# jyjblrd/Low-Cost-Mocap

Hardware: AMD Instinct MI355X
Metric: triangulated 3D markers/sec at 8 cams x 16 markers (higher is better)
Workload: dtype f64

## Files before the change

### low-cost-mocap_amd/csrc/frame_bb.hip

```cpp
#include "mocap_device.hpp"
#include "kernels.hpp"
#include <cstdlib>
#include "frame_common.hpp"

namespace mocap {

constexpr int kBBThreads = 256;
constexpr int kBBWaves = kBBThreads / 64;
constexpr int kBBRecs = kBBThreads + 64;

constexpr int bb_wg_per_cu(int RL) { return RL == 48 ? 5 : 4; }
constexpr int kBBLdsSlack = 1024;
struct BBLayout {
  size_t bxy, bxy_nx, cnt_nx, bt, rbound, seedkey, slot_key, claimw, recs, rpk, scr, scr_bytes, goff, gcnt, outslot, boff, bnb, seedgh, slot_g, cnt,
      misc, bpl, nh, hits, act, root_blob, root_cam, nact, bnl, bv, bcache, bpk, total;
  int ncache;
  __host__ __device__ static size_t al(size_t x, size_t a) { return (x + a - 1) / a * a; }
  __host__ __device__ BBLayout(int C, int M, int R, int CW, int wg_per_cu) {
    size_t o = 0;
    auto take = [&](size_t bytes, size_t a) {
      o = al(o, a);
      const size_t at = o;
      o += bytes;
      return at;
    };
    bxy = take(sizeof(float2) * (size_t)C * M, 16);
    bxy_nx = take(sizeof(float2) * (size_t)C * M, 16);
    cnt_nx = take(4 * (size_t)C, 4);
    bt = take(sizeof(double) * 10 * ((size_t)C * M + 1), 16);
    rbound = take(8 * (size_t)R, 8);
    claimw = take(8 * (size_t)C, 8);
    scr = seedkey = take(8 * (size_t)R, 8);
    slot_key = take(8 * (size_t)kBBWaves * R, 8);
    recs = take(8 * (size_t)kBBRecs, 8);
    rpk = take(8 * (size_t)kBBRecs * CW, 8);
    seedgh = take(4 * (size_t)R, 4);
    slot_g = take(4 * (size_t)kBBWaves * R, 4);
    scr_bytes = o - scr;
    goff = take(4 * (size_t)(R + 1), 4);
    gcnt = take(4 * (size_t)R, 4);
    outslot = take(4 * (size_t)R, 4);
    boff = take(4 * (size_t)(R + 1), 4);
    bnb = take(4 * (size_t)R, 4);
    cnt = take(4 * (size_t)C, 4);
    misc = take(4 * 16, 4);
    bpl = take(2 * (size_t)R, 2);
    nh = take((size_t)R * C, 1);
    hits = take((size_t)R * C * M, 1);
    act = take((size_t)R * C, 1);
    root_blob = take((size_t)R, 1);
    root_cam = take((size_t)R, 1);
    nact = take((size_t)R, 1);
    bnl = take((size_t)R, 1);
    bv = take((size_t)R, 1);
    bcache = take(0, 8);
    ncache = 0;
    const size_t per_entry = 8 + 8 * (size_t)CW;
    for (int per_cu = wg_per_cu; per_cu >= 1; per_cu--) {
      const size_t lim = ((size_t)160 * 1024 / per_cu - kBBLdsSlack) / 256 * 256;
      if (lim >= o + per_entry * 64) {
        const size_t n = (lim - o) / per_entry;
        ncache = (int)(n > 1024 ? 1024 : n);
        break;
      }
    }
    o += 8 * (size_t)ncache;
    bpk = o;
    o += 8 * (size_t)CW * ncache;
    total = al(o, 16);
  }
};

static int bb_fixed_slots(int C, int M, int R) {
  const char* e = getenv("MOCAP_BB_FIXED_LAYOUT");
  if (e && e[0] == '0') return 0;
  if (C == 8 && M == 16 && R <= 48) return 48;
  if (C == 8 && M == 16 && R <= 64) return 64;
  return 0;
}
static int frame_bb_root_slots(int C, int M, int R) {
  const int f = bb_fixed_slots(C, M, R);
  return f ? f : R;
}
size_t frame_bb_lds_bytes(int C, int M, int R) { return BBLayout(C, M, frame_bb_root_slots(C, M, R), C <= 8 ? 1 : 2, bb_wg_per_cu(bb_fixed_slots(C, M, R))).total; }
static size_t frame_bb_lds_bytes_min(int C, int M, int R) {
  const BBLayout L(C, M, frame_bb_root_slots(C, M, R), C <= 8 ? 1 : 2, bb_wg_per_cu(bb_fixed_slots(C, M, R)));
  return L.total - (8 + 8 * (size_t)(C <= 8 ? 1 : 2)) * (size_t)L.ncache;
}
bool frame_bb_fits(int C, int M, int R) {
  return C >= 2 && C <= 16 && M >= 1 && M <= 64 && R >= 1 && R <= 255 && frame_bb_lds_bytes_min(C, M, R) <= (size_t)128 * 1024;
}

template <int CW>
struct Packed {
  unsigned long long w[CW];
  __device__ __forceinline__ void clear() {
#pragma unroll
    for (int k = 0; k < CW; k++) w[k] = ~0ull;
  }
  __device__ __forceinline__ void set(int c, uint32_t idx) {
    if (CW == 1)
      w[0] ^= (unsigned long long)(idx ^ 0xFFu) << (8 * c);
    else
      w[c >> 3] ^= (unsigned long long)(idx ^ 0xFFu) << (8 * (c & 7));
  }
  __device__ __forceinline__ uint32_t get(int c) const {
    return CW == 1 ? (uint32_t)(w[0] >> (8 * c)) & 0xFFu : (uint32_t)(w[c >> 3] >> (8 * (c & 7))) & 0xFFu;
  }
};

template <int CT, bool PERK = false>
struct BBCamTables {
  const double* base;
  static constexpr int C = CT;
  static constexpr int kPq = PERK ? 12 * CT * CT : 12 * CT;
  __device__ __forceinline__ ctab_t pq(size_t off) const { return as_ctab(base + off); }
  __device__ __forceinline__ ctab_t rt(size_t off) const { return as_ctab(base + kPq + off); }
  __device__ __forceinline__ ctab_t k4(size_t off) const { return as_ctab(base + kPq + 12 * CT + off); }
  __device__ __forceinline__ const double* f() const { return base + kPq + 16 * CT; }
};
template <bool PERK>
struct BBCamTables<0, PERK> {
  const double* base;
  int C;
  __device__ __forceinline__ ctab_t pq(size_t off) const { return as_ctab(base + off); }
  __device__ __forceinline__ ctab_t rt(size_t off) const { return as_ctab(base + (PERK ? 12 * C * C : 12 * C) + off); }
  __device__ __forceinline__ ctab_t k4(size_t off) const { return as_ctab(base + (PERK ? 12 * C * C + 12 * C : 24 * C) + off); }
  __device__ __forceinline__ const double* f() const { return base + (PERK ? 12 * C * C + 16 * C : 28 * C); }
};

enum { kPrioEval = 0, kPrioSeed = 1, kPrioPhase = 2, kPrioSerial = 3 };
template <int P>
__device__ __forceinline__ void bb_prio() {
  __builtin_amdgcn_s_setprio(P);
}

template <bool F32R, int CW, int CT, int ML, int RL, bool PERK = false>
struct BBState {
  static constexpr int T = kBBThreads, W = kBBWaves;
  const FrameArgs& p;
  BBCamTables<CT, PERK> cv;
  const int C_, M, R, RS;
  int tid, lane, wave;
  __device__ __forceinline__ void fresh_tid() {
    int t = tid;
    asm volatile("" : "+v"(t));
    tid = t;
    lane = t & 63;
    wave = t >> 6;
  }
  __device__ __forceinline__ int cn() const { return CT > 0 ? CT : C_; }
  double* bt;
  float2 *bxy, *bxy_nx;
  int32_t* cnt_nx;
  unsigned long long *rbound, *seedkey, *slot_key, *claimw, *rpk;
  struct BRec { uint32_t gh, rs; };
  BRec* recs;
  uint32_t *goff, *gcnt, *boff, *bnb, *seedgh, *slot_g;
  int32_t *outslot, *cnt, *misc;
  uint16_t* bpl;
  uint8_t *nh, *hits, *act, *root_blob, *root_cam, *nact, *bnl, *bv;
  float2* bcache;
  unsigned long long* bpk;
  int ncache;
  unsigned char* scr;
  size_t scr_bytes;
  static constexpr unsigned long long kInfBits = 0x7ff0000000000000ull;

  __device__ BBState(const FrameArgs& p_, unsigned char* smem)
      : p(p_), C_(p_.cv.C), M(ML > 0 ? ML : p_.M), R(p_.K_max), RS(RL > 0 ? RL : p_.K_max), tid(threadIdx.x), lane(threadIdx.x & 63), wave(threadIdx.x >> 6) {
    const int C = cn();
    {
      const unsigned long long ta = (unsigned long long)(uintptr_t)p_.cv.Pq;
      uint32_t tlo = (uint32_t)__builtin_amdgcn_readfirstlane((int)(uint32_t)ta);
      uint32_t thi = (uint32_t)__builtin_amdgcn_readfirstlane((int)(uint32_t)(ta >> 32));
      asm volatile("" : "+s"(tlo), "+s"(thi));
      cv.base = (const double*)(uintptr_t)(((unsigned long long)thi << 32) | tlo);
      if constexpr (CT == 0) cv.C = C;
    }
    const BBLayout L(C, M, RS, CW, bb_wg_per_cu(RL));
    bt = (double*)(smem + L.bt);
    bxy = (float2*)(smem + L.bxy);
    bxy_nx = (float2*)(smem + L.bxy_nx);
    cnt_nx = (int32_t*)(smem + L.cnt_nx);
    rbound = (unsigned long long*)(smem + L.rbound);
    seedkey = (unsigned long long*)(smem + L.seedkey);
    slot_key = (unsigned long long*)(smem + L.slot_key);
    claimw = (unsigned long long*)(smem + L.claimw);
    recs = (BRec*)(smem + L.recs);
    rpk = (unsigned long long*)(smem + L.rpk);
    goff = (uint32_t*)(smem + L.goff);
    gcnt = (uint32_t*)(smem + L.gcnt);
    outslot = (int32_t*)(smem + L.outslot);
    boff = (uint32_t*)(smem + L.boff);
    bnb = (uint32_t*)(smem + L.bnb);
    seedgh = (uint32_t*)(smem + L.seedgh);
    slot_g = (uint32_t*)(smem + L.slot_g);
    cnt = (int32_t*)(smem + L.cnt);
    misc = (int32_t*)(smem + L.misc);
    bpl = (uint16_t*)(smem + L.bpl);
    nh = (uint8_t*)(smem + L.nh);
    hits = (uint8_t*)(smem + L.hits);
    act = (uint8_t*)(smem + L.act);
    root_blob = (uint8_t*)(smem + L.root_blob);
    root_cam = (uint8_t*)(smem + L.root_cam);
    nact = (uint8_t*)(smem + L.nact);
    bnl = (uint8_t*)(smem + L.bnl);
    bv = (uint8_t*)(smem + L.bv);
    scr = smem + L.scr;
    scr_bytes = L.scr_bytes;
    bcache = (float2*)(smem + L.bcache);
    bpk = (unsigned long long*)(smem + L.bpk);
    ncache = L.ncache;
  }

  struct Line { double a, b, c, den, rden; };
  __device__ __forceinline__ Line epiline(int r, int i) const { return epiline_of(root_cam[r], root_blob[r], i); }
  __device__ __forceinline__ Line epiline_of(int rc, int rb, int i) const {
    const int C = cn();
    const double* Fm = cv.f() + 9 * ((size_t)rc * C + i);
    const float2 rp = bxy[(size_t)rc * M + rb];
    const double x = (double)rp.x, y = (double)rp.y;
    double a = Fm[0] * x + Fm[1] * y + Fm[2];
    double b = Fm[3] * x + Fm[4] * y + Fm[5];
    double c = Fm[6] * x + Fm[7] * y + Fm[8];
    double nu = a * a + b * b;
    nu = nu != 0.0 ? 1.0 / sqrt(nu) : 1.0;
    a *= nu;
    b *= nu;
    c *= nu;
    if (F32R) {
      a = (double)(float)a;
      b = (double)(float)b;
      c = (double)(float)c;
    }
    Line L;
    L.a = a;
    L.b = b;
    L.c = c;
    L.den = sqrt(a * a + b * b);
    L.rden = recip_refined(L.den);
    return L;
  }

  template <bool CHAIN>
  __device__ __forceinline__ unsigned long long match_pairs(const Line& mine, int pair_r, int pair_i, int n_pairs, int gs_shift,
                                                            int cam = 0, int Mi_chain = 0) {
    const int C = cn();
    const int GS = 1 << gs_shift, PPS = 64 >> gs_shift;
    const int k = lane & (GS - 1), q = lane >> gs_shift;
    const int gl0 = lane & ~(GS - 1);
    const unsigned long long gall = gs_shift == 6 ? ~0ull : ((1ull << GS) - 1ull);
    unsigned long long claims = 0ull;
    for (int s0 = 0; s0 < n_pairs; s0 += PPS) {
      const int src = s0 + q;
      const bool has = src < n_pairs;
      const int sl = has ? src : 0;
      const double la = __shfl(mine.a, sl), lb = __shfl(mine.b, sl), lc = __shfl(mine.c, sl);
      const double lden = __shfl(mine.den, sl), lrden = __shfl(mine.rden, sl);
      const int r = __shfl(pair_r, sl);
      const int i = CHAIN ? cam : __shfl(pair_i, sl);
      const int Mi = has ? (CHAIN ? Mi_chain : cnt[i]) : 0;
      const bool valid = k < Mi;
      float2 pt = make_float2(0.f, 0.f);
      double d = 0.0;
      bool hit = false;
      if (valid) {
        pt = bxy[(size_t)i * M + k];
        const double num = fabs(la * (double)pt.x + lb * (double)pt.y + lc);
        d = div_by(num, lden, lrden);
        hit = d < p.gate_px;
      }
      const unsigned long long wm = __ballot(hit);
      const unsigned long long gm = (wm >> gl0) & gall;
      int rank = 0;
      const unsigned int dlo = (unsigned int)__double_as_longlong(d), dhi = (unsigned int)(__double_as_longlong(d) >> 32);
      for (unsigned long long mm = wm; mm;) {
        const int j = __ffsll((long long)mm) - 1;
        mm &= mm - 1;
        const double dj = __longlong_as_double(((long long)__builtin_amdgcn_readlane((int)dhi, j) << 32) |
                                               (unsigned int)__builtin_amdgcn_readlane((int)dlo, j));
        const bool mine_grp = (j & ~(GS - 1)) == gl0 && j != lane;
        rank += (hit && mine_grp && (dj < d || (dj == d && j < lane))) ? 1 : 0;
      }
      if (hit) hits[((size_t)r * C + i) * M + rank] = (uint8_t)k;
      const unsigned long long g0 = (__ballot(hit && rank == 0) >> gl0) & gall;
      bool same = false;
      if (valid && g0) {
        const float2 p0 = bxy[(size_t)i * M + (__ffsll((long long)g0) - 1)];
        same = pt.x == p0.x && pt.y == p0.y;
      }
      const unsigned long long cw = __ballot(same);
      if (CHAIN) {
        for (int sh = 0; sh < 64; sh += GS) claims |= (cw >> sh) & gall;
      }
      if (has && k == 0) {
        nh[(size_t)r * C + i] = (uint8_t)__popcll(gm);
        if (!CHAIN) {
          const unsigned long long cm = (cw >> gl0) & gall;
          if (cm) atomicOr(&claimw[i], cm);
        }
      }
    }
    return claims;
  }

  __device__ __forceinline__ void prefetch_lds(int64_t frame) const {
    const int C = cn();
    const float* src = p.blobs + (size_t)frame * C * M * 2;
    const int n_dw = C * M * 2;
    for (int base = wave * 64; base < n_dw; base += T)
      if (base + lane < n_dw)
        __builtin_amdgcn_global_load_lds((const __attribute__((address_space(1))) void*)(src + base + lane),
                                         (__attribute__((address_space(3))) void*)((float*)bxy_nx + base), 4, 0, 0);
    if (wave == 0 && lane < C)
      __builtin_amdgcn_global_load_lds((const __attribute__((address_space(1))) void*)(p.counts + (size_t)frame * C + lane),
                                       (__attribute__((address_space(3))) void*)cnt_nx, 4, 0, 0);
  }
  __device__ __forceinline__ void stage(int64_t frame) {
    fresh_tid();
    const int C = cn();
    float2* t = bxy;
    bxy = bxy_nx;
    bxy_nx = t;
    if (tid < C) {
      const int n = cnt_nx[tid];
      cnt[tid] = n < 0 ? 0 : (n > M ? M : n);
      claimw[tid] = 0ull;
    }
    if (tid == 0) {
      misc[MI_STATUS] = 0;
      misc[MI_OMAX] = 0;
    }
  }

  __device__ void match() {
    fresh_tid();
    const int C = cn();
    __syncthreads();
    int gs_shift = 0;
    while ((1 << gs_shift) < M) gs_shift++;
    const int n0 = cnt[0] < R ? cnt[0] : R;
    {
      for (int r = tid; r < n0; r += T) {
        root_cam[r] = 0;
        root_blob[r] = (uint8_t)r;
      }
      if (tid == 0 && cnt[0] > R) misc[MI_STATUS] |= MOCAP_ST_ROOT_OVERFLOW_;
    }
    __syncthreads();
    auto U_of = [&](int j) {
      const int n = cnt[j];
      return ~claimw[j] & (n >= 64 ? ~0ull : ((1ull << n) - 1ull));
    };
    int n_prov = 0, n_ppairs = 0;
    bool pre = false;
    uint8_t* nh_s = nullptr;
    uint8_t* hits_s = nullptr;
    unsigned long long* pclaim = (unsigned long long*)scr;
    {
      int Mmax = 0;
      for (int c = 1; c < C; c++) Mmax = cnt[c] > Mmax ? cnt[c] : Mmax;
#pragma nounroll
      for (int stage_ = 0; stage_ < 2; stage_++) {
        const int stage = __builtin_amdgcn_readfirstlane(stage_);
        int NP = n0 * (C - 1);
        if (stage == 1) {
          block_sync_lds();
          for (int j = 1; j < C; j++) {
            const int np = __popcll(U_of(j));
            n_prov += np;
            n_ppairs += np * (C - 1 - j);
          }
          pre = n_prov <= 64 && (size_t)n_prov * C * (8 + 1 + (size_t)M) <= scr_bytes;
          if (!pre) break;
          nh_s = (uint8_t*)(pclaim + (size_t)n_prov * C);
          hits_s = nh_s + (size_t)n_prov * C;
          NP = n_ppairs;
        }
        for (int base = wave * 64; base < NP; base += W * 64) {
          const int pi = base + lane;
          const bool have = pi < NP;
          int r = 0, i = 1, Mi = 0;
          Line L = {0, 0, 0, 1, 1};
          if (have) {
            if (stage == 0) {
              r = pi / (C - 1);
              i = 1 + (pi - r * (C - 1));
              L = epiline(r, i);
            } else {
              int j = 1, acc = 0, pb = 0, span = C - 2;
              unsigned long long U = 0ull;
              for (; j <= C - 2; j++) {
                span = C - 1 - j;
                U = U_of(j);
                const int nj = __popcll(U) * span;
                if (pi < acc + nj) break;
                acc += nj;
                pb += __popcll(U);
              }
              uint32_t ord, off;
              divmod_tiny((uint32_t)(pi - acc), (uint32_t)span, ord, off);
              for (uint32_t t = 0; t < ord; t++) U &= U - 1;
              const int k = __ffsll((long long)U) - 1;
              i = j + 1 + (int)off;
              r = pb + (int)ord;
              L = epiline_of(j, k, i);
            }
            Mi = cnt[i];
          }
          const float2* pts = bxy + (size_t)i * M;
          auto dist = [&](int k) {
            const float2 pt = pts[k];
            return div_by(fabs(L.a * (double)pt.x + L.b * (double)pt.y + L.c), L.den, L.rden);
          };
          unsigned long long hm = 0ull;
#pragma unroll 4
          for (int k = 0; k < Mmax; k++)
            if (k < Mi && dist(k) < p.gate_px) hm |= 1ull << k;
          uint8_t* nhp = stage == 0 ? nh : nh_s;
          uint8_t* hl = (stage == 0 ? hits : hits_s) + ((size_t)r * C + i) * M;
          if (have) nhp[(size_t)r * C + i] = (uint8_t)__popcll(hm);
          unsigned long long rem = hm, claim = 0ull;
          int pos = 0;
          float2 p0 = make_float2(0.f, 0.f);
          while (__ballot(rem != 0ull)) {
            if (rem) {
              double bd = __builtin_huge_val();
              int bk = 0;
              for (unsigned long long t = rem; t; t &= t - 1) {
                const int k = __ffsll((long long)t) - 1;
                const double d = dist(k);
                if (d < bd) {
                  bd = d;
                  bk = k;
                }
              }
              hl[pos] = (uint8_t)bk;
              if (pos == 0) {
                p0 = pts[bk];
                for (unsigned long long t = hm; t; t &= t - 1) {
                  const int k = __ffsll((long long)t) - 1;
                  const float2 q = pts[k];
                  if (q.x == p0.x && q.y == p0.y) claim |= 1ull << k;
                }
              }
              rem &= ~(1ull << bk);
              pos++;
            }
          }
          if (stage == 0) {
            if (claim) atomicOr(&claimw[i], claim);
          } else if (have) {
            pclaim[(size_t)r * C + i] = claim;
          }
        }
      }
    }
    const int NL = M * ((C - 1) * (C - 2) / 2);
    const bool spec = F32R && (size_t)NL * 20 + 8 <= scr_bytes;
    double* sp_den = (double*)scr;
    float* sp_abc = (float*)(sp_den + NL);
    auto sp_base = [&](int j) { return M * ((j - 1) * (C - 1) - (j - 1) * j / 2); };
    if (spec && !pre) {
      int tot = 0;
      for (int j = 1; j <= C - 2; j++) {
        const int n = cnt[j];
        const unsigned long long U = ~claimw[j] & (n >= 64 ? ~0ull : ((1ull << n) - 1ull));
        tot += __popcll(U) * (C - 1 - j);
      }
      for (int l = tid; l < tot; l += T) {
        int j = 1, acc = 0, span = C - 2;
        unsigned long long U = 0ull;
        for (; j <= C - 2; j++) {
          const int n = cnt[j];
          U = ~claimw[j] & (n >= 64 ? ~0ull : ((1ull << n) - 1ull));
          span = C - 1 - j;
          const int nj = __popcll(U) * span;
          if (l < acc + nj) break;
          acc += nj;
        }
        uint32_t ord, off;
        divmod_tiny((uint32_t)(l - acc), (uint32_t)span, ord, off);
        for (uint32_t t = 0; t < ord; t++) U &= U - 1;
        const int k = __ffsll((long long)U) - 1, i = j + 1 + (int)off;
        const int ll = sp_base(j) + k * span + (int)off;
        const Line L = epiline_of(j, k, i);
        sp_den[ll] = L.den;
        sp_abc[3 * ll + 0] = (float)L.a;
        sp_abc[3 * ll + 1] = (float)L.b;
        sp_abc[3 * ll + 2] = (float)L.c;
      }
    }
    __syncthreads();
    fresh_tid();
    if (wave == 0) bb_prio<kPrioSerial>();
    if (wave == 0 && pre) {
      int jp = 0, kp = 0;
      if (lane < n_prov) {
        int acc = 0;
        unsigned long long U = 0ull;
        for (jp = 1; jp < C; jp++) {
          U = U_of(jp);
          const int np = __popcll(U);
          if (lane < acc + np) break;
          acc += np;
        }
        for (int t = 0; t < lane - acc; t++) U &= U - 1;
        kp = __ffsll((long long)U) - 1;
      }
      bool real = false;
      for (int i = 1; i < C; i++) {
        wave_lds_sync();
        if (lane < n_prov && jp == i) {
          real = !((claimw[i] >> kp) & 1ull);
          if (real)
            for (int c = i + 1; c < C; c++) {
              const unsigned long long m = pclaim[(size_t)lane * C + c];
              if (m) atomicOr(&claimw[c], m);
            }
        }
      }
      const unsigned long long rm = __ballot(real);
      const int rank = __popcll(rm & ((1ull << lane) - 1ull));
      int n_roots = n0 + __popcll(rm);
      if (real && n0 + rank < R) {
        root_cam[n0 + rank] = (uint8_t)jp;
        root_blob[n0 + rank] = (uint8_t)kp;
        bnl[rank] = (uint8_t)lane;
      }
      if (lane == 0) {
        if (n_roots > R) {
          misc[MI_STATUS] |= MOCAP_ST_ROOT_OVERFLOW_;
          n_roots = R;
        }
        misc[MI_NROOTS] = n_roots;
      }
    } else if (wave == 0) {
      const int cntL = lane < C ? cnt[lane] : 0;
      const unsigned long long clmL = lane < C ? claimw[lane] : 0ull;
      int nr_cam = 0, nr_blob = 0;
      int n_roots = n0;
      bool over = false;
      for (int i = 1; i < C; i++) {
        const int Mi = __builtin_amdgcn_readlane(cntL, i);
        unsigned long long claimed = ((unsigned long long)(unsigned int)__builtin_amdgcn_readlane((int)(clmL >> 32), i) << 32) |
                                     (unsigned int)__builtin_amdgcn_readlane((int)clmL, i);
        const int n_new = n_roots - n0;
        for (int base = 0; base < n_new; base += 64) {
          const int l = base + lane;
          const bool have = l < n_new;
          int j = nr_cam, k = nr_blob;
          if (base) {
            wave_lds_sync();
            j = have ? root_cam[n0 + l] : 0;
            k = have ? root_blob[n0 + l] : 0;
          }
          Line L = {0, 0, 0, 1, 1};
          if (have) {
            if (spec) {
              const int ll = sp_base(j) + k * (C - 1 - j) + (i - j - 1);
              L.a = (double)sp_abc[3 * ll + 0];
              L.b = (double)sp_abc[3 * ll + 1];
              L.c = (double)sp_abc[3 * ll + 2];
              L.den = sp_den[ll];
              L.rden = recip_refined(L.den);
            } else {
              L = epiline_of(j, k, i);
            }
          }
          claimed |= match_pairs<true>(L, n0 + l, i, (n_new - base < 64) ? n_new - base : 64, gs_shift, i, Mi);
        }
        const bool flag = lane < Mi && !((claimed >> lane) & 1ull);
        const unsigned long long mask = __ballot(flag);
        const int pos = __popcll(mask & ((1ull << lane) - 1ull));
        if (flag) {
          const int rr = n_roots + pos;
          if (rr < R) {
            root_cam[rr] = (uint8_t)i;
            root_blob[rr] = (uint8_t)lane;
          }
        }
        int slot = n_new;
        for (unsigned long long mm = mask; mm; slot++) {
          const int jb = __ffsll((long long)mm) - 1;
          mm &= mm - 1;
          if (lane == slot) {
            nr_cam = i;
            nr_blob = jb;
          }
        }
        n_roots += __popcll(mask);
        if (n_roots > R) {
          over = true;
          n_roots = R;
        }
      }
      if (lane == 0) {
        if (over) misc[MI_STATUS] |= MOCAP_ST_ROOT_OVERFLOW_;
        misc[MI_NROOTS] = n_roots;
      }
    } else {
      float om = 0.0f;
      for (int i = tid - 64; i < C * M; i += T - 64) {
        const int c = i / M, k = i - c * M;
        if (k < cnt[c]) {
          const float2 v = bxy[i];
          om = fmaxf(om, fmaxf(fabsf(v.x), fabsf(v.y)));
          double Bc[10];
          dlt_contribution(Bc, cv.pq(PERK ? 12 * (c * C + c) : 12 * c), (double)v.x, (double)v.y);
#pragma unroll
          for (int e = 0; e < 10; e++) bt[(size_t)i * 10 + e] = Bc[e];
        }
      }
      if (om > 0.0f) atomicMax(&misc[MI_OMAX], __float_as_int(om));
      if (tid == 64) {
        const int it = q_add(&p.q.counters[QC_NEXT_FRAME], 1);
        misc[MI_NEXT] = it < frame_count(p) ? it : -1;
      }
    }
    bb_prio<kPrioPhase>();
    __syncthreads();
    if (pre) {
      const int n_new = misc[MI_NROOTS] - n0;
      for (int idx = tid; idx < n_new * C; idx += T) {
        const int q = idx / C, c = idx - q * C;
        const int r = n0 + q, ps = bnl[q];
        if (c > (int)root_cam[r]) {
          const int n = nh_s[(size_t)ps * C + c];
          nh[(size_t)r * C + c] = (uint8_t)n;
          const uint8_t* src = hits_s + ((size_t)ps * C + c) * M;
          uint8_t* dst = hits + ((size_t)r * C + c) * M;
          for (int t = 0; t < n; t++) dst[t] = src[t];
        }
      }
      __syncthreads();
    }

    fresh_tid();
    const int nroots = misc[MI_NROOTS];
    for (int r = tid; r < nroots; r += T) {
      const int rc = root_cam[r];
      unsigned long long total = 1;
      int views = 1, na = 0;
      bool over = false;
      for (int c = rc + 1; c < C; c++) {
        const unsigned n = nh[(size_t)r * C + c];
        if (n > 1) act[(size_t)r * C + na++] = (uint8_t)c;
        if (n) {
          views++;
          total *= n;
          if (total > (unsigned long long)p.G_cap) {
            over = true;
            total = 1;
          }
        }
      }
      if (over) atomicOr(&misc[MI_STATUS], MOCAP_ST_CAND_OVERFLOW_);
      nact[r] = (uint8_t)na;
      bv[r] = (uint8_t)views;
      rbound[r] = kInfBits;
      const uint32_t g = (views > 1 && !over) ? (uint32_t)total : 0u;
      gcnt[r] = g;
      {
        const uint8_t* a = act + (size_t)r * C;
        uint32_t pl = 1, nb = 1;
        int nl = 0;
        while (nl < na && pl < (uint32_t)p.bb_pl) pl *= nh[(size_t)r * C + a[nl++]];
        for (int k = nl; k < na; k++) nb *= nh[(size_t)r * C + a[k]];
        bpl[r] = (uint16_t)pl;
        bnl[r] = (uint8_t)nl;
        bnb[r] = g ? nb : 0u;
        seedkey[r] = 0ull;
        seedgh[r] = 0xFFFFFFFFu;
      }
    }
    for (int s = tid; s < W * RS; s += T) {
      slot_key[s] = ~0ull;
      slot_g[s] = 0xFFFFFFFFu;
    }
    if (tid == 0) misc[MI_BBCTR] = misc[MI_BBCTR2] = 0;
    __syncthreads();
    if (wave == 0) bb_prio<kPrioSerial>();
    if (wave == 0) {
      uint32_t carry = 0, bcarry = 0;
      int slots = 0;
      for (int base = 0; base < nroots; base += 64) {
        const int r = base + lane;
        const uint32_t g = r < nroots ? gcnt[r] : 0u;
        const uint32_t nb = r < nroots ? bnb[r] : 0u;
        const uint32_t incl = wave_inclusive_scan(g, lane);
        const uint32_t bincl = wave_inclusive_scan(nb, lane);
        const unsigned long long nz = __ballot(g != 0u);
        if (r < nroots) {
          goff[r] = carry + incl - g;
          boff[r] = bcarry + bincl - nb;
          outslot[r] = g ? slots + __popcll(nz & ((1ull << lane) - 1ull)) : -1;
        }
        carry += (uint32_t)__builtin_amdgcn_readlane((int)incl, 63);
        bcarry += (uint32_t)__builtin_amdgcn_readlane((int)bincl, 63);
        slots += __popcll(nz);
      }
      if (lane == 0) {
        goff[nroots] = carry;
        boff[nroots] = bcarry;
        misc[MI_NOUT] = slots;
        misc[MI_G] = misc[MI_STATUS] ? 0 : (int32_t)carry;
      }
    }
    bb_prio<kPrioPhase>();
    __syncthreads();
  }

  __device__ __forceinline__ void add_view(double (&B)[10], int c, uint32_t k, int j) const {
    if (PERK && j != c) {
      const float2 w = bxy[(size_t)c * M + k];
      double Bc[10];
      dlt_contribution(Bc, cv.base + 12 * ((size_t)j * cn() + c), (double)w.x, (double)w.y);
#pragma unroll
      for (int e = 0; e < 10; e++) B[e] = B[e] + Bc[e];
    } else {
      const double* t = bt + ((size_t)c * M + k) * 10;
#pragma unroll
      for (int e = 0; e < 10; e++) B[e] = B[e] + t[e];
    }
  }

  template <bool WITH_B>
  __device__ __forceinline__ int group_matrix(int r, uint32_t rem, int skip, double (&B)[10], Packed<CW>& pk) const {
    const int C = cn();
    const int rc = root_cam[r];
    const uint8_t* nhr = nh + (size_t)r * C;
    const uint8_t* hr = hits + (size_t)r * C * M;
    pk.clear();
    int v = 0, ka = 0;
    int j = 0;
    if (WITH_B) {
#pragma unroll
      for (int e = 0; e < 10; e++) B[e] = 0.0;
    }
    for (int c = 0; c < C; c++) {
      uint32_t k = 0xFFu;
      bool seen = false;
      if (c == rc) {
        k = root_blob[r];
        seen = true;
      } else if (c > rc) {
        const uint32_t n = nhr[c];
        seen = n != 0;
        if (n == 1) {
          k = hr[(size_t)c * M];
        } else if (n > 1) {
          if (ka >= skip) {
            uint32_t qd, dgt;
            if (rem < 8192u) divmod_tiny(rem, n, qd, dgt); else
            divmod_small(rem, n, qd, dgt);
            rem = qd;
            k = hr[(size_t)c * M + dgt];
          }
          ka++;
        }
      }
      if (k != 0xFFu) {
        if (WITH_B) add_view(B, c, k, j);
        v++;
        pk.set(c, k);
      }
      if (PERK) j += seen ? 1 : 0;
    }
    return v;
  }

  __device__ __forceinline__ int fetch_candidate(uint32_t lo, uint32_t i, int& r, uint32_t& gl, Packed<CW>& pk, double (&B)[10]) const {
    const int C = cn();
    const BRec rec = recs[lo];
    r = (int)(rec.rs & 0xFFu);
#pragma unroll
    for (int k = 0; k < CW; k++) pk.w[k] = rpk[(size_t)lo * CW + k];
    if (rec.rs >> 31) {
      gl = rec.gh;
    } else {
      uint32_t rem = i - (rec.rs >> 8);
      gl = rec.gh * (uint32_t)bpl[r] + rem;
      const uint8_t* a = act + (size_t)r * C;
      const int nl = bnl[r];
      for (int k = 0; k < nl; k++) {
        const int c = a[k];
        uint32_t qd, dgt;
        divmod_tiny(rem, nh[(size_t)r * C + c], qd, dgt);
        rem = qd;
        pk.set(c, hits[((size_t)r * C + c) * M + dgt]);
      }
    }
#pragma unroll
    for (int ee = 0; ee < 10; ee++) B[ee] = 0.0;
    if constexpr (PERK) {
      int j = 0;
#pragma unroll CT > 0 ? CT : 1
      for (int c = 0; c < C; c++) {
        const uint32_t k = pk.get(c);
        if (k != 0xFFu) add_view(B, c, k, j++);
      }
    } else {
#pragma unroll CT > 0 ? CT : 1
      for (int c = 0; c < C; c++) {
        const uint32_t k = pk.get(c);
        const double* t = bt + (size_t)(k != 0xFFu ? (uint32_t)c * (uint32_t)M + k : (uint32_t)C * (uint32_t)M) * 10;
#pragma unroll
        for (int ee = 0; ee < 10; ee++) B[ee] = B[ee] + t[ee];
      }
    }
    return bv[r];
  }

  __device__ void search(bool bound_tests) {
    fresh_tid();
    const int C = cn();
    (void)C;
    const int nroots = misc[MI_NROOTS];
    int32_t* ctr = &misc[MI_BBCTR];
    int32_t* ctr_other = &misc[MI_BBCTR2];
    const double inf = __builtin_huge_val();
    EigCut ec;
    {
      const double om = (double)__int_as_float(misc[MI_OMAX]);
      ec.p3max2 = p.p3max2;
      ec.o2slack = (1100.0 * 0x1p-46) * (om * om);
    }
    const double c0[3] = {p.bb_c0[0], p.bb_c0[1], p.bb_c0[2]};
    const uint32_t nblocks = boff[nroots];
    auto root_of_block = [&](uint32_t b_first_of_wave, uint32_t b) {
      return coop_last_le([&](int r) { return boff[r]; }, nroots, b_first_of_wave, b, lane);
    };
    auto push_block = [&](int r, uint32_t gh, const Packed<CW>& pk) {
      const uint32_t old = (uint32_t)atomicAdd(ctr, (int32_t)(((uint32_t)bpl[r] << 10) | 1u));
      const uint32_t slot = old & 0x3FFu;
      BRec rec;
      rec.gh = gh;
      rec.rs = (uint32_t)r | ((old >> 10) << 8);
      recs[slot] = rec;
#pragma unroll
      for (int k = 0; k < CW; k++) rpk[(size_t)slot * CW + k] = pk.w[k];
    };
    auto rec_start = [&](int k) { return (recs[k].rs & 0x7FFFFFFFu) >> 8; };
    auto dropped = [&](int r, double s1, double tr) {
      const int vf = bv[r];
      const double bound = __longlong_as_double((long long)rbound[r]);
      const double limit = bound * (double)(2 * vf) * (1.0 + 0x1p-40);
      const double limit_adj = fma(1.002, limit, (double)(2 * vf) * ec.o2slack);
      return s1 * fma(2e-12, tr, p.p3max2c * limit_adj) < 1.0;
    };
    if (bound_tests) {
      bb_prio<kPrioSeed>();
      int my_r = -1;
      uint32_t my_gh = 0;
      unsigned long long my_key = 0ull;
      Packed<CW> my_pk;
      my_pk.clear();
      for (uint32_t s0 = 0; s0 < nblocks; s0 += T) {
        const uint32_t b = s0 + (uint32_t)tid;
        if (s0 + (uint32_t)(wave * 64) >= nblocks) continue;
        const int r = root_of_block(s0 + (uint32_t)(wave * 64), b < nblocks ? b : nblocks - 1);
        if (b < nblocks) {
          const uint32_t gh = b - boff[r];
          double B[10], tr = 0.0;
          Packed<CW> pk;
          const int v = group_matrix<true>(r, gh, bnl[r], B, pk);
          double s1d = __builtin_huge_val();
          float s1 = 0.0f;
          if (v >= 2) {
            s1d = eigcut_s1_shifted(B, c0, tr);
            s1 = (float)fmin(s1d, 3e38);
          }
          if (b < (uint32_t)ncache) {
            bcache[b] = make_float2(__double2float_ru(s1d), __double2float_ru(tr));
#pragma unroll
            for (int k = 0; k < CW; k++) bpk[(size_t)b * CW + k] = pk.w[k];
          }
          my_key = ((unsigned long long)__float_as_uint(s1) << 32) | (unsigned long long)(0xFFFFFFFFu - gh);
          my_r = r;
          my_gh = gh;
          my_pk = pk;
          atomicMax(&seedkey[r], my_key);
        }
      }
      __syncthreads();
      if (nblocks <= (uint32_t)T) {
        if (my_r >= 0 && seedkey[my_r] == my_key) {
          seedgh[my_r] = my_gh;
          push_block(my_r, my_gh, my_pk);
        }
      } else
      for (int r = tid; r < nroots; r += T) {
        if (bnb[r]) {
          const uint32_t gh = 0xFFFFFFFFu - (uint32_t)seedkey[r];
          seedgh[r] = gh;
          seedkey[r] = 0ull;
          double B[10];
          Packed<CW> pk;
          group_matrix<false>(r, gh, bnl[r], B, pk);
          push_block(r, gh, pk);
        }
      }
      bb_prio<kPrioEval>();
      __syncthreads();
    }
    uint32_t b0 = 0;
    fresh_tid();
    while (true) {
      const uint32_t cv_ = (uint32_t)*ctr;
      const uint32_t ns = cv_ & 0x3FFu, ne = cv_ >> 10;
      const bool blocks_left = b0 < nblocks;
      const bool full = ns > (uint32_t)(kBBRecs - T);
      if (ns && (full || !blocks_left || ne >= (uint32_t)p.bb_flush)) {
        for (uint32_t i0 = 0; i0 < ne; i0 += T) {
          const uint32_t i = i0 + (uint32_t)tid;
          const bool have = i < ne;
          double e = inf, X[3] = {0, 0, 0};
          int r = 0;
          uint32_t gl = 0;
          uint32_t lo = 0;
          if (i0 + (uint32_t)(wave * 64) < ne)
            lo = (uint32_t)coop_last_le(rec_start, (int)ns, i0 + (uint32_t)(wave * 64), have ? i : ne - 1, lane);
          if (have) {
            Packed<CW> pk;
            double B[10];
            const int v = fetch_candidate(lo, i, r, gl, pk, B);
            auto obs_p = [&](int c, double& x, double& y) -> bool {
              const uint32_t k = pk.get(c);
              if (k == 0xFFu) return false;
              const float2 w = bxy[(size_t)c * M + k];
              x = (double)w.x;
              y = (double)w.y;
              return true;
            };
            const double bound = __longlong_as_double((long long)rbound[r]);
            solve_and_score<!PERK, true, F32R, false>(cv, B, v, obs_p, X, e, bound * (double)(2 * v) * (1.0 + 0x1p-40), ec);
#ifdef MOCAP_DEBUG_EIGCHECK
            if (!(e < inf)) {
              double B2[10], X2[3], e2;
#pragma unroll
              for (int ee = 0; ee < 10; ee++) B2[ee] = 0.0;
              int j2 = 0;
              for (int c = 0; c < C; c++) {
                const uint32_t k = pk.get(c);
                if (k != 0xFFu) add_view(B2, c, k, j2++);
              }
              solve_and_score<!PERK, true, F32R>(cv, B2, v, obs_p, X2, e2);
              atomicAdd(&p.status[p.n_frames], 1);
              if (e2 <= bound) printf("EIGCHECK candidate: root %d g %u bound %.17g true %.17g\n", r, gl, bound, e2);
            }
#endif
          }
          const bool fin = e < inf;
          const unsigned long long key = fin ? (unsigned long long)__double_as_longlong(e) : kInfBits;
          const uint32_t gword = (gl << 1) | ((e != e) ? 1u : 0u);
          const int ss = wave * RS + r;
          if (fin) atomicMin(&rbound[r], key);
          const bool want = have && (key < slot_key[ss] || (key == slot_key[ss] && gword < slot_g[ss]));
          if (__ballot(want)) {
            unsigned long long old = 0;
            if (want) old = atomicMin(&slot_key[ss], key);
            wave_lds_sync();
            const bool holder = want && slot_key[ss] == key;
            if (holder && old > key) slot_g[ss] = 0xFFFFFFFFu;
            wave_lds_sync();
            if (holder) atomicMin(&slot_g[ss], gword);
            wave_lds_sync();
          }
        }
        __syncthreads();
        if (tid == 0) *ctr = 0;
        {
          int32_t* t = ctr;
          ctr = ctr_other;
          ctr_other = t;
        }
        continue;
      }
      if (!blocks_left) break;
      const uint32_t b = b0 + (uint32_t)tid;
      const uint32_t bw = b0 + (uint32_t)(wave * 64);
      b0 += T;
      int r = 0;
      if (bw < nblocks) r = root_of_block(bw, b < nblocks ? b : nblocks - 1);
      bool do_push = false;
      uint32_t gh = 0;
      Packed<CW> pk;
      pk.clear();
      if (b < nblocks) {
        gh = b - boff[r];
        if (gh != seedgh[r]) {
          double B[10], tr;
          bool survive = true;
          if (bound_tests && b < (uint32_t)ncache) {
            const float2 sc = bcache[b];
            survive = !dropped(r, (double)sc.x, (double)sc.y);
#pragma unroll
            for (int k = 0; k < CW; k++) pk.w[k] = bpk[(size_t)b * CW + k];
          } else if (bound_tests) {
            const int v = group_matrix<true>(r, gh, bnl[r], B, pk);
            if (v >= 2) {
              const double s1 = eigcut_s1_shifted(B, c0, tr);
              survive = !dropped(r, s1, tr);
            }
          } else {
            group_matrix<false>(r, gh, bnl[r], B, pk);
          }
          do_push = survive;
#ifdef MOCAP_DEBUG_EIGCHECK
          if (!survive) {
            const double bound = __longlong_as_double((long long)rbound[r]);
            const uint32_t pl = bpl[r];
            for (uint32_t l = 0; l < pl; l++) {
              double B2[10], X2[3], e2 = inf;
              Packed<CW> pk2;
              const int v2 = group_matrix<true>(r, gh * pl + l, 0, B2, pk2);
              auto obs2 = [&](int c, double& x, double& y) -> bool {
                const uint32_t k = pk2.get(c);
                if (k == 0xFFu) return false;
                const float2 w = bxy[(size_t)c * M + k];
                x = (double)w.x;
                y = (double)w.y;
                return true;
              };
              solve_and_score<!PERK, true, F32R>(cv, B2, v2, obs2, X2, e2);
              atomicAdd(&p.status[p.n_frames + 1], 1);
              if (e2 <= bound) printf("EIGCHECK block: root %d block %u candidate %u bound %.17g true %.17g\n", r, gh, l, bound, e2);
            }
          }
#endif
        }
      }
      __syncthreads();
      if (do_push) push_block(r, gh, pk);
      __syncthreads();
    }
    __syncthreads();
  }

  __device__ bool root_winner(int r, double& eb, uint32_t& gb) const {
    if (!gcnt[r]) return false;
    unsigned long long kb = ~0ull;
    uint32_t gw = 0xFFFFFFFFu;
    for (int w = 0; w < W; w++) {
      const int s = w * RS + r;
      const unsigned long long k = slot_key[s];
      const uint32_t g = slot_g[s];
      if (k < kb || (k == kb && g < gw)) {
        kb = k;
        gw = g;
      }
    }
    if (kb == ~0ull) return false;
    gb = gw >> 1;
    eb = kb != kInfBits ? __longlong_as_double((long long)kb)
                        : ((gw & 1u) ? __longlong_as_double(0x7ff8000000000000ll) : __builtin_huge_val());
    return true;
  }

  __device__ void write_point(int64_t frame, int r, double e, uint32_t gl) const {
    const int C = cn();
    const size_t o = (size_t)frame * R + outslot[r];
    p.err[o] = e;
    double B[10];
#pragma unroll
    for (int ee = 0; ee < 10; ee++) B[ee] = 0.0;
    uint32_t rem = gl;
    const int rc = root_cam[r];
    int16_t* co = p.corr + o * C;
    int j = 0;
    for (int c = 0; c < C; c++) {
      int16_t s = -1;
      if (c == rc) {
        s = (int16_t)root_blob[r];
      } else if (c > rc) {
        const uint32_t n = nh[(size_t)r * C + c];
        if (n) {
          uint32_t qd = rem, dgt = 0;
          if (n > 1) {
            if (rem < 8192u) divmod_tiny(rem, n, qd, dgt); else
            divmod_small(rem, n, qd, dgt);
          }
          s = (int16_t)hits[((size_t)r * C + c) * M + dgt];
          rem = qd;
        }
      }
      co[c] = s;
      if (s >= 0) add_view(B, c, (uint32_t)s, j++);
    }
    double X[3];
    solve_point(B, X);
    store_point(p, o, X);
  }
};

template <bool F32R, int CW, int CT, int ML, int RL>
__global__ __launch_bounds__(kBBThreads, bb_wg_per_cu(RL)) void frame_bb_kernel(FrameArgs p) {
  extern __shared__ __attribute__((aligned(16))) unsigned char smem[];
#define BB_STATE BBState<F32R, CW, CT, ML, RL>
#include "frame_bb_body.inc"
#undef BB_STATE
}

template <bool F32R, int CW, int CT, int ML, int RL>
__global__ __launch_bounds__(kBBThreads, bb_wg_per_cu(RL)) void frame_bb_calib_kernel(FrameArgs p) {
  extern __shared__ __attribute__((aligned(16))) unsigned char smem[];
#define BB_STATE BBState<F32R, CW, CT, ML, RL, true>
#include "frame_bb_body.inc"
#undef BB_STATE
}

int frame_bb_wg_per_cu_cap(int C, int M, int R) { return bb_wg_per_cu(bb_fixed_slots(C, M, R)); }
size_t frame_bb_ws_bytes(int) { return 0; }

hipError_t launch_frame_bb(const FrameArgs& a, int grid, hipStream_t stream) {
  const size_t lds = frame_bb_lds_bytes(a.cv.C, a.M, a.K_max);
  const size_t nPq = a.cv.uniformK ? (size_t)12 * a.cv.C : (size_t)12 * a.cv.C * a.cv.C;
  if (a.cv.RT != a.cv.Pq + nPq || a.cv.K4 != a.cv.RT + 12 * a.cv.C || a.cv.F != a.cv.K4 + 4 * a.cv.C) return hipErrorInvalidValue;
  void (*k)(FrameArgs);
  const bool f32 = a.cv.f32_rounding != 0;
  const int fixed = bb_fixed_slots(a.cv.C, a.M, a.K_max);
  if (fixed && fixed != 48 && fixed != 64) return hipErrorInvalidValue;
#define BB_PICK(KERNEL)                                                                             \
  (fixed == 48       ? (f32 ? KERNEL<true, 1, 8, 16, 48> : KERNEL<false, 1, 8, 16, 48>)             \
   : fixed == 64     ? (f32 ? KERNEL<true, 1, 8, 16, 64> : KERNEL<false, 1, 8, 16, 64>)             \
   : a.cv.C == 8     ? (f32 ? KERNEL<true, 1, 8, 0, 0> : KERNEL<false, 1, 8, 0, 0>)                 \
   : a.cv.C <= 8     ? (f32 ? KERNEL<true, 1, 0, 0, 0> : KERNEL<false, 1, 0, 0, 0>)                 \
                     : (f32 ? KERNEL<true, 2, 0, 0, 0> : KERNEL<false, 2, 0, 0, 0>))
  k = a.cv.uniformK ? BB_PICK(frame_bb_kernel) : BB_PICK(frame_bb_calib_kernel);
#undef BB_PICK
  if (lds > 48 * 1024) {
    hipError_t e = hipFuncSetAttribute((const void*)k, hipFuncAttributeMaxDynamicSharedMemorySize, (int)lds);
    if (e != hipSuccess) return e;
  }
  hipLaunchKernelGGL(k, dim3(grid), dim3(kBBThreads), lds, stream, a);
  return hipGetLastError();
}

}
```

### low-cost-mocap_amd/csrc/frame_bb_body.inc

```
  BB_STATE st(p, smem);
  const int tid = threadIdx.x;
  const FrameQueues& q = p.q;
  if (tid == 0) {
    const int it = q_add(&q.counters[QC_NEXT_FRAME], 1);
    st.misc[MI_ITEM] = it < frame_count(p) ? it : -1;
  }
  if (tid < 10) st.bt[(size_t)st.cn() * st.M * 10 + tid] = 0.0;
  __syncthreads();
  int item = st.misc[MI_ITEM];
  if (item >= 0) st.prefetch_lds(item);
  wait_own_stores();
  __syncthreads();
  while (item >= 0) {
    const int64_t frame = item;
    bb_prio<kPrioPhase>();
    st.stage(frame);
    st.match();
    bb_prio<kPrioEval>();
    const int next = st.misc[MI_NEXT];
    if (next >= 0) st.prefetch_lds(next);
    if (tid == 0) {
      const int status = st.misc[MI_STATUS];
      p.n_out[frame] = status ? 0 : st.misc[MI_NOUT];
      p.status[frame] = status;
      if (p.n_cand) p.n_cand[frame] = st.misc[MI_G];
    }
    const uint32_t G = (uint32_t)st.misc[MI_G];
    if (G) {
      st.search(G >= (uint32_t)p.bb_min_g);
      bb_prio<kPrioPhase>();
      const int nroots = st.misc[MI_NROOTS];
      st.fresh_tid();
      for (int r = st.tid; r < nroots; r += kBBThreads) {
        if (st.outslot[r] < 0) continue;
        double e;
        uint32_t gl;
        if (st.root_winner(r, e, gl)) st.write_point(frame, r, e, gl);
      }
    }
    wait_own_stores();
    bb_prio<kPrioEval>();
    __syncthreads();
    item = next;
  }
  if (tid == 0 && q_add(&q.counters[QC_EXITED], 1) == (int)gridDim.x - 1)
    for (int c = 0; c < QC_COUNT; c++) q_store(&q.counters[c], 0);
```

Baseline: 562.0 million.

## Split seed block into fine sub-blocks with per-sub-block eigen bound tests

When a root's last leading camera has at most four hits, the seed block is split into finer sub-blocks, one per hit of that camera. Each sub-block gets its own eigen lower bound, computed by a quad of lanes, and only the best one is pushed as the seed. The other sub-blocks are queued as extra bound tests that can be pruned against the seed's result. A forced flush after the seed round tightens bounds early. This aims to cut candidate evaluations, at the cost of extra eigen-bound work, LDS space and more complex record encoding.

```diff
diff --git a/low-cost-mocap_amd/csrc/frame_bb.hip b/low-cost-mocap_amd/csrc/frame_bb.hip
--- a/low-cost-mocap_amd/csrc/frame_bb.hip
+++ b/low-cost-mocap_amd/csrc/frame_bb.hip
@@ -8,11 +8,12 @@
 constexpr int kBBThreads = 256;
 constexpr int kBBWaves = kBBThreads / 64;
 constexpr int kBBRecs = kBBThreads + 64;
+constexpr int kBBSubCap = 4;
 
 constexpr int bb_wg_per_cu(int RL) { return RL == 48 ? 5 : 4; }
 constexpr int kBBLdsSlack = 1024;
 struct BBLayout {
-  size_t bxy, bxy_nx, cnt_nx, bt, rbound, seedkey, slot_key, claimw, recs, rpk, scr, scr_bytes, goff, gcnt, outslot, boff, bnb, seedgh, slot_g, cnt,
+  size_t bxy, bxy_nx, cnt_nx, bt, rbound, seedkey, slot_key, claimw, recs, rpk, scr, scr_bytes, bsub, gcnt, outslot, boff, bnb, seedgh, slot_g, cnt,
       misc, bpl, nh, hits, act, root_blob, root_cam, nact, bnl, bv, bcache, bpk, total;
   int ncache;
   __host__ __device__ static size_t al(size_t x, size_t a) { return (x + a - 1) / a * a; }
@@ -30,14 +31,14 @@
     bt = take(sizeof(double) * 10 * ((size_t)C * M + 1), 16);
     rbound = take(8 * (size_t)R, 8);
     claimw = take(8 * (size_t)C, 8);
-    scr = seedkey = take(8 * (size_t)R, 8);
+    scr = seedkey = take(16 * (size_t)R, 8);
     slot_key = take(8 * (size_t)kBBWaves * R, 8);
     recs = take(8 * (size_t)kBBRecs, 8);
     rpk = take(8 * (size_t)kBBRecs * CW, 8);
     seedgh = take(4 * (size_t)R, 4);
     slot_g = take(4 * (size_t)kBBWaves * R, 4);
     scr_bytes = o - scr;
-    goff = take(4 * (size_t)(R + 1), 4);
+    bsub = take(4 * (size_t)R, 4);
     gcnt = take(4 * (size_t)R, 4);
     outslot = take(4 * (size_t)R, 4);
     boff = take(4 * (size_t)(R + 1), 4);
@@ -129,6 +130,14 @@
   __device__ __forceinline__ const double* f() const { return base + (PERK ? 12 * C * C + 16 * C : 28 * C); }
 };
 
+__device__ __forceinline__ uint32_t quad_max(uint32_t v) {
+  uint32_t o = (uint32_t)__builtin_amdgcn_update_dpp(0, (int)v, 0xB1, 0xF, 0xF, true);
+  v = v > o ? v : o;
+  o = (uint32_t)__builtin_amdgcn_update_dpp(0, (int)v, 0x4E, 0xF, 0xF, true);
+  return v > o ? v : o;
+}
+__device__ __forceinline__ uint32_t quad_min(uint32_t v) { return ~quad_max(~v); }
+
 enum { kPrioEval = 0, kPrioSeed = 1, kPrioPhase = 2, kPrioSerial = 3 };
 template <int P>
 __device__ __forceinline__ void bb_prio() {
@@ -156,7 +165,7 @@
   unsigned long long *rbound, *seedkey, *slot_key, *claimw, *rpk;
   struct BRec { uint32_t gh, rs; };
   BRec* recs;
-  uint32_t *goff, *gcnt, *boff, *bnb, *seedgh, *slot_g;
+  uint32_t *bsub, *gcnt, *boff, *bnb, *seedgh, *slot_g;
   int32_t *outslot, *cnt, *misc;
   uint16_t* bpl;
   uint8_t *nh, *hits, *act, *root_blob, *root_cam, *nact, *bnl, *bv;
@@ -189,7 +198,7 @@
     claimw = (unsigned long long*)(smem + L.claimw);
     recs = (BRec*)(smem + L.recs);
     rpk = (unsigned long long*)(smem + L.rpk);
-    goff = (uint32_t*)(smem + L.goff);
+    bsub = (uint32_t*)(smem + L.bsub);
     gcnt = (uint32_t*)(smem + L.gcnt);
     outslot = (int32_t*)(smem + L.outslot);
     boff = (uint32_t*)(smem + L.boff);
@@ -664,14 +673,19 @@
       gcnt[r] = g;
       {
         const uint8_t* a = act + (size_t)r * C;
-        uint32_t pl = 1, nb = 1;
+        uint32_t pl = 1, nb = 1, sub = 1, nlast = 1;
         int nl = 0;
-        while (nl < na && pl < (uint32_t)p.bb_pl) pl *= nh[(size_t)r * C + a[nl++]];
+        while (nl < na && pl < (uint32_t)p.bb_pl) {
+          nlast = nh[(size_t)r * C + a[nl++]];
+          sub = pl;
+          pl *= nlast;
+        }
         for (int k = nl; k < na; k++) nb *= nh[(size_t)r * C + a[k]];
         bpl[r] = (uint16_t)pl;
         bnl[r] = (uint8_t)nl;
         bnb[r] = g ? nb : 0u;
-        seedkey[r] = 0ull;
+        bsub[r] = (nl >= 1 && sub >= 2u && nlast <= (uint32_t)kBBSubCap) ? (sub | (nlast << 16)) : 0u;
+        seedkey[2 * r] = 0ull;
         seedgh[r] = 0xFFFFFFFFu;
       }
     }
@@ -693,7 +707,6 @@
         const uint32_t bincl = wave_inclusive_scan(nb, lane);
         const unsigned long long nz = __ballot(g != 0u);
         if (r < nroots) {
-          goff[r] = carry + incl - g;
           boff[r] = bcarry + bincl - nb;
           outslot[r] = g ? slots + __popcll(nz & ((1ull << lane) - 1ull)) : -1;
         }
@@ -702,7 +715,6 @@
         slots += __popcll(nz);
       }
       if (lane == 0) {
-        goff[nroots] = carry;
         boff[nroots] = bcarry;
         misc[MI_NOUT] = slots;
         misc[MI_G] = misc[MI_STATUS] ? 0 : (int32_t)carry;
@@ -777,13 +789,12 @@
     r = (int)(rec.rs & 0xFFu);
 #pragma unroll
     for (int k = 0; k < CW; k++) pk.w[k] = rpk[(size_t)lo * CW + k];
-    if (rec.rs >> 31) {
-      gl = rec.gh;
-    } else {
-      uint32_t rem = i - (rec.rs >> 8);
-      gl = rec.gh * (uint32_t)bpl[r] + rem;
+    {
+      const uint32_t fine = rec.rs >> 31;
+      uint32_t rem = i - ((rec.rs & 0x7FFFFFFFu) >> 8);
+      gl = rec.gh * (fine ? bsub[r] & 0xFFFFu : (uint32_t)bpl[r]) + rem;
       const uint8_t* a = act + (size_t)r * C;
-      const int nl = bnl[r];
+      const int nl = (int)bnl[r] - (int)fine;
       for (int k = 0; k < nl; k++) {
         const int c = a[k];
         uint32_t qd, dgt;
@@ -813,13 +824,15 @@
     return bv[r];
   }
 
-  __device__ void search(bool bound_tests) {
+  __device__ void search(bool bound_tests_) {
     fresh_tid();
     const int C = cn();
     (void)C;
-    const int nroots = misc[MI_NROOTS];
-    int32_t* ctr = &misc[MI_BBCTR];
-    int32_t* ctr_other = &misc[MI_BBCTR2];
+    const bool bound_tests = __builtin_amdgcn_readfirstlane((int)bound_tests_) != 0;
+    const int nroots = __builtin_amdgcn_readfirstlane(misc[MI_NROOTS]);
+    static_assert(MI_BBCTR2 == MI_BBCTR + 2, "the queue counters: misc[MI_BBCTR + 2 k]");
+    int cur = 0;
+    auto ctr = [&] { return &misc[MI_BBCTR + 2 * cur]; };
     const double inf = __builtin_huge_val();
     EigCut ec;
     {
@@ -828,16 +841,17 @@
       ec.o2slack = (1100.0 * 0x1p-46) * (om * om);
     }
     const double c0[3] = {p.bb_c0[0], p.bb_c0[1], p.bb_c0[2]};
-    const uint32_t nblocks = boff[nroots];
+    const uint32_t nblocks = (uint32_t)__builtin_amdgcn_readfirstlane((int)boff[nroots]);
     auto root_of_block = [&](uint32_t b_first_of_wave, uint32_t b) {
       return coop_last_le([&](int r) { return boff[r]; }, nroots, b_first_of_wave, b, lane);
     };
-    auto push_block = [&](int r, uint32_t gh, const Packed<CW>& pk) {
-      const uint32_t old = (uint32_t)atomicAdd(ctr, (int32_t)(((uint32_t)bpl[r] << 10) | 1u));
+    auto push_block = [&](int r, uint32_t gh, const Packed<CW>& pk, bool fine) {
+      const uint32_t n = fine ? bsub[r] & 0xFFFFu : (uint32_t)bpl[r];
+      const uint32_t old = (uint32_t)atomicAdd(ctr(), (int32_t)((n << 10) | 1u));
       const uint32_t slot = old & 0x3FFu;
       BRec rec;
       rec.gh = gh;
-      rec.rs = (uint32_t)r | ((old >> 10) << 8);
+      rec.rs = (uint32_t)r | ((old >> 10) << 8) | (fine ? 0x80000000u : 0u);
       recs[slot] = rec;
 #pragma unroll
       for (int k = 0; k < CW; k++) rpk[(size_t)slot * CW + k] = pk.w[k];
@@ -850,13 +864,29 @@
       const double limit_adj = fma(1.002, limit, (double)(2 * vf) * ec.o2slack);
       return s1 * fma(2e-12, tr, p.p3max2c * limit_adj) < 1.0;
     };
+#ifdef MOCAP_DEBUG_EIGCHECK
+    auto eigcheck_dropped = [&](int r, uint32_t gh, uint32_t pl) {
+      const double bound = __longlong_as_double((long long)rbound[r]);
+      for (uint32_t l = 0; l < pl; l++) {
+        double B2[10], X2[3], e2 = inf;
+        Packed<CW> pk2;
+        const int v2 = group_matrix<true>(r, gh * pl + l, 0, B2, pk2);
+        auto obs2 = [&](int c, double& x, double& y) -> bool {
+          const uint32_t k = pk2.get(c);
+          if (k == 0xFFu) return false;
+          const float2 w = bxy[(size_t)c * M + k];
+          x = (double)w.x;
+          y = (double)w.y;
+          return true;
+        };
+        solve_and_score<!PERK, true, F32R>(cv, B2, v2, obs2, X2, e2);
+        atomicAdd(&p.status[p.n_frames + 1], 1);
+        if (e2 <= bound) printf("EIGCHECK block: root %d block %u of %u candidates, candidate %u bound %.17g true %.17g\n", r, gh, pl, l, bound, e2);
+      }
+    };
+#endif
     if (bound_tests) {
       bb_prio<kPrioSeed>();
-      int my_r = -1;
-      uint32_t my_gh = 0;
-      unsigned long long my_key = 0ull;
-      Packed<CW> my_pk;
-      my_pk.clear();
       for (uint32_t s0 = 0; s0 < nblocks; s0 += T) {
         const uint32_t b = s0 + (uint32_t)tid;
         if (s0 + (uint32_t)(wave * 64) >= nblocks) continue;
@@ -877,29 +907,41 @@
 #pragma unroll
             for (int k = 0; k < CW; k++) bpk[(size_t)b * CW + k] = pk.w[k];
           }
-          my_key = ((unsigned long long)__float_as_uint(s1) << 32) | (unsigned long long)(0xFFFFFFFFu - gh);
-          my_r = r;
-          my_gh = gh;
-          my_pk = pk;
-          atomicMax(&seedkey[r], my_key);
+          atomicMax(&seedkey[2 * r], ((unsigned long long)__float_as_uint(s1) << 32) | (unsigned long long)(0xFFFFFFFFu - gh));
         }
       }
       __syncthreads();
-      if (nblocks <= (uint32_t)T) {
-        if (my_r >= 0 && seedkey[my_r] == my_key) {
-          seedgh[my_r] = my_gh;
-          push_block(my_r, my_gh, my_pk);
-        }
-      } else
-      for (int r = tid; r < nroots; r += T) {
-        if (bnb[r]) {
-          const uint32_t gh = 0xFFFFFFFFu - (uint32_t)seedkey[r];
-          seedgh[r] = gh;
-          seedkey[r] = 0ull;
-          double B[10];
-          Packed<CW> pk;
-          group_matrix<false>(r, gh, bnl[r], B, pk);
-          push_block(r, gh, pk);
+      for (int i0 = 0; i0 < nroots * 4; i0 += T) {
+        const int idx = i0 + tid, r = idx >> 2;
+        const uint32_t d = (uint32_t)idx & 3u;
+        bool mine = false, fine = false;
+        uint32_t gh = 0, ghs = 0, sbits = 0, tbits = 0;
+        Packed<CW> pk;
+        pk.clear();
+        if (r < nroots && bnb[r]) {
+          gh = 0xFFFFFFFFu - (uint32_t)seedkey[2 * r];
+          const uint32_t nlast = (bsub[r] >> 16) & 0xFFu;
+          fine = nlast != 0u;
+          mine = fine ? d < nlast : d == 0u;
+          if (mine) {
+            ghs = fine ? gh * nlast + d : gh;
+            double B[10], tr = 0.0;
+            const int v = group_matrix<true>(r, ghs, (int)bnl[r] - (fine ? 1 : 0), B, pk);
+            double s1d = __builtin_huge_val();
+            if (fine && v >= 2) s1d = eigcut_s1_shifted(B, c0, tr);
+            sbits = __float_as_uint(__double2float_ru(s1d));
+            tbits = __float_as_uint(__double2float_ru(tr));
+          }
+        }
+        const uint32_t smax = quad_max(sbits), tmax = quad_max(tbits);
+        const uint32_t dsel = quad_min(mine && fine && sbits == smax ? d : 4u);
+        if (mine) {
+          if (fine) ((uint32_t*)&seedkey[2 * r])[d] = d == dsel ? tmax : sbits;
+          if (!fine || d == dsel) {
+            seedgh[r] = gh;
+            if (fine) bsub[r] |= dsel << 24;
+            push_block(r, ghs, pk, fine);
+          }
         }
       }
       bb_prio<kPrioEval>();
@@ -908,12 +950,15 @@
     uint32_t b0 = 0;
     fresh_tid();
     while (true) {
-      const uint32_t cv_ = (uint32_t)*ctr;
+      const uint32_t cv_ = (uint32_t)__builtin_amdgcn_readfirstlane(*ctr());
       const uint32_t ns = cv_ & 0x3FFu, ne = cv_ >> 10;
-      const bool blocks_left = b0 < nblocks;
+      const uint32_t ntests = nblocks + (bound_tests ? (uint32_t)nroots * 4u : 0u);
+      const bool blocks_left = b0 < ntests;
       const bool full = ns > (uint32_t)(kBBRecs - T);
-      if (ns && (full || !blocks_left || ne >= (uint32_t)p.bb_flush)) {
+      const bool seed_round = bound_tests && b0 == 0 && (uint32_t)__builtin_amdgcn_readfirstlane(misc[MI_G]) > (uint32_t)T;
+      if (ns && (seed_round || full || !blocks_left || ne >= (uint32_t)p.bb_flush)) {
         for (uint32_t i0 = 0; i0 < ne; i0 += T) {
+          fresh_tid();
           const uint32_t i = i0 + (uint32_t)tid;
           const bool have = i < ne;
           double e = inf, X[3] = {0, 0, 0};
@@ -970,24 +1015,40 @@
           }
         }
         __syncthreads();
-        if (tid == 0) *ctr = 0;
-        {
-          int32_t* t = ctr;
-          ctr = ctr_other;
-          ctr_other = t;
-        }
+        if (tid == 0) *ctr() = 0;
+        cur ^= 1;
         continue;
       }
       if (!blocks_left) break;
+      fresh_tid();
       const uint32_t b = b0 + (uint32_t)tid;
       const uint32_t bw = b0 + (uint32_t)(wave * 64);
       b0 += T;
       int r = 0;
       if (bw < nblocks) r = root_of_block(bw, b < nblocks ? b : nblocks - 1);
-      bool do_push = false;
+      bool do_push = false, fine = false;
       uint32_t gh = 0;
       Packed<CW> pk;
       pk.clear();
+      if (b >= nblocks && b < ntests) {
+        r = (int)((b - nblocks) >> 2);
+        const uint32_t d = (b - nblocks) & 3u, bs = bnb[r] ? bsub[r] : 0u;
+        const uint32_t nlast = (bs >> 16) & 0xFFu, dsel = bs >> 24;
+        if (d < nlast && d != dsel) {
+          const float* sb = (const float*)&seedkey[2 * r];
+          fine = true;
+          gh = seedgh[r] * nlast + d;
+          do_push = !dropped(r, (double)sb[d], (double)sb[dsel]);
+          if (do_push) {
+            double B[10];
+            group_matrix<false>(r, gh, (int)bnl[r] - 1, B, pk);
+          }
+#ifdef MOCAP_DEBUG_EIGCHECK
+          else
+            eigcheck_dropped(r, gh, bs & 0xFFFFu);
+#endif
+        }
+      } else
       if (b < nblocks) {
         gh = b - boff[r];
         if (gh != seedgh[r]) {
@@ -1009,31 +1070,12 @@
           }
           do_push = survive;
 #ifdef MOCAP_DEBUG_EIGCHECK
-          if (!survive) {
-            const double bound = __longlong_as_double((long long)rbound[r]);
-            const uint32_t pl = bpl[r];
-            for (uint32_t l = 0; l < pl; l++) {
-              double B2[10], X2[3], e2 = inf;
-              Packed<CW> pk2;
-              const int v2 = group_matrix<true>(r, gh * pl + l, 0, B2, pk2);
-              auto obs2 = [&](int c, double& x, double& y) -> bool {
-                const uint32_t k = pk2.get(c);
-                if (k == 0xFFu) return false;
-                const float2 w = bxy[(size_t)c * M + k];
-                x = (double)w.x;
-                y = (double)w.y;
-                return true;
-              };
-              solve_and_score<!PERK, true, F32R>(cv, B2, v2, obs2, X2, e2);
-              atomicAdd(&p.status[p.n_frames + 1], 1);
-              if (e2 <= bound) printf("EIGCHECK block: root %d block %u candidate %u bound %.17g true %.17g\n", r, gh, l, bound, e2);
-            }
-          }
+          if (!survive) eigcheck_dropped(r, gh, bpl[r]);
 #endif
         }
       }
       __syncthreads();
-      if (do_push) push_block(r, gh, pk);
+      if (do_push) push_block(r, gh, pk, fine);
       __syncthreads();
     }
     __syncthreads();
diff --git a/low-cost-mocap_amd/csrc/frame_bb_body.inc b/low-cost-mocap_amd/csrc/frame_bb_body.inc
--- a/low-cost-mocap_amd/csrc/frame_bb_body.inc
+++ b/low-cost-mocap_amd/csrc/frame_bb_body.inc
@@ -40,8 +40,8 @@
     }
     wait_own_stores();
     bb_prio<kPrioEval>();
+    item = st.misc[MI_NEXT];
     __syncthreads();
-    item = next;
   }
   if (tid == 0 && q_add(&q.counters[QC_EXITED], 1) == (int)gridDim.x - 1)
     for (int c = 0; c < QC_COUNT; c++) q_store(&q.counters[c], 0);
```

Result: no change. 567.4 million, median of 6 (+1.0%).
